# Deltares/xugrid

Hardware: AMD Instinct MI355X
Metric: target cells regridded/s (OverlapRegridder 1M->1M tri, weights + mean apply) (higher is better)
Workload: dtype f64; 1 GPU; BASELINE config 2: ~1M-triangle jittered-lattice Delaunay source -> ~1M-triangle target (seed 1, rotated 30 deg, scaled 0.7), OverlapRegridder area-weighted mean, K=1; target_faces=999660, candidate_pairs=6677422, nnz=4052965, parallelism=1 GPU

## Files before the change

include/xugrid_amd.h:

```cpp
#ifndef XUGRID_AMD_H
#define XUGRID_AMD_H

#include <stdint.h>

#ifdef __cplusplus
extern "C" {
#endif

#define XR_OK 0
#define XR_ERR_INVALID (-1)
#define XR_ERR_NO_DEVICE (-2)
#define XR_ERR_HIP (-3)
#define XR_ERR_LIMIT (-4)

#define XR_MEAN 0
#define XR_HARMONIC_MEAN 1
#define XR_GEOMETRIC_MEAN 2
#define XR_SUM 3
#define XR_MINIMUM 4
#define XR_MAXIMUM 5
#define XR_MODE 6
#define XR_PERCENTILE 7
#define XR_FIRST_ORDER_CONSERVATIVE 8
#define XR_MAX_OVERLAP 9
#define XR_SELECT 10

#define XR_F64 0
#define XR_F32 1
#define XR_I32 2

#define XR_MAX_FACE_NODES 32

typedef struct xr_mesh xr_mesh;
typedef struct xr_csr xr_csr;
typedef struct xr_outer xr_outer;

const char *xr_last_error(void);
int xr_device_count(int *count);
int xr_init(int device);
int xr_current_device(int *device);
int xr_trim_pool(void);
int xr_version(void);
int xr_set_stream(void *hip_stream, int external, int async_dev);
int xr_set_async(int on);
int xr_set_option(const char *name, int64_t value);
int xr_get_option(const char *name, int64_t *value);
int xr_host_copy(void *dst, const void *src, int64_t bytes);
int xr_host_interleave2(const double *x, int64_t x_stride, const double *y, int64_t y_stride, int64_t n, double *out_xy);

int xr_mesh_create(const double *node_xy, int64_t n_node, const void *faces, int faces_itemsize,
                   int64_t n_face, int64_t n_max_node, int64_t fill_value, xr_mesh **out);
int xr_mesh_create_dev(const double *node_xy_dev, int64_t n_node, const void *faces_dev, int faces_itemsize,
                       int64_t n_face, int64_t n_max_node, int64_t fill_value, xr_mesh **out);
int xr_mesh_create_rectilinear(const double *x_vertices, int64_t nx, const double *y_vertices, int64_t ny,
                               xr_mesh **out);
int xr_mesh_destroy(xr_mesh *mesh);
int xr_mesh_info(const xr_mesh *mesh, int64_t *n_node, int64_t *n_face, int64_t *n_max_node);
int xr_mesh_device_bytes(const xr_mesh *mesh, int64_t *bytes);
int xr_mesh_prepare(xr_mesh *mesh);
int xr_mesh_build_index(xr_mesh *mesh);
int xr_mesh_invalidate(xr_mesh *mesh);
int xr_mesh_area(xr_mesh *mesh, double *area_out);
int xr_mesh_centroids(xr_mesh *mesh, double *centroids_out);
int xr_mesh_faces(xr_mesh *mesh, int64_t *faces_out);
int xr_mesh_download(xr_mesh *mesh, double *node_xy_out, int64_t *faces_out);
int xr_mesh_triangulate(xr_mesh *mesh, xr_mesh **out);
int xr_mesh_triangle_face_dev(const xr_mesh *triangles, int64_t *index_dev);
int xr_mesh_circumcenters_dev(xr_mesh *mesh, double *out_dev);
int xr_mesh_perimeter_dev(xr_mesh *mesh, double *out_dev);
int xr_mesh_face_bounds_dev(xr_mesh *mesh, double *out_dev);

int xr_overlap(xr_mesh *tree, xr_mesh *query, int relative, xr_csr **out);
int xr_overlap_stats(const xr_mesh *tree, int64_t *n_candidates);
int xr_overlap_apply_dev(xr_mesh *tree, xr_mesh *query, int relative, int method, double percentile,
                         const void *source_dev, int source_dtype, int64_t K, double *out_dev, xr_csr **out);

int xr_locate_points(xr_mesh *mesh, const double *points, int64_t n, double tolerance,
                     int64_t *face_index_out);
int xr_locate_raster(xr_mesh *mesh, const double *x, int64_t nx, const double *y, int64_t ny,
                     double tolerance, int64_t *face_index_out);
int xr_barycentric(xr_mesh *mesh, const double *points, int64_t n, double tolerance,
                   int64_t *face_index_out, double *weights_out);

int xr_replace_interpolated_weights(const double *vertices, int64_t n_vertex, const int64_t *faces, int64_t n_face,
                                    int64_t m, const int64_t *face_index, double *weights, int64_t n,
                                    const int64_t *node_to_node_map, int64_t n_map);

int xr_locate_csr(xr_mesh *tree, xr_mesh *query, const double *points, int64_t n, double tolerance,
                  xr_csr **out);

int xr_barycentric_csr(xr_mesh *voronoi, xr_mesh *source, xr_mesh *query, const double *points,
                       int64_t n, double tolerance, const int64_t *vertex_face,
                       const int64_t *node_to_node_map, int64_t n_extra, xr_csr **out);
int xr_barycentric_csr_tail(xr_mesh *voronoi, xr_mesh *source, xr_mesh *query, const double *points, int64_t n,
                            double tolerance, int64_t n_identity, const int64_t *vertex_face_tail,
                            const int64_t *node_to_node_map, int64_t n_extra, int tree_order, xr_csr **out);

typedef struct xr_points xr_points;
int xr_locate_flags_begin(xr_mesh *source, xr_mesh *query, const double *points, int64_t n, xr_points **out);
int xr_points_destroy(xr_points *points);
int xr_barycentric_csr_points(xr_mesh *voronoi, xr_mesh *source, xr_points *points, double tolerance, int64_t n_identity,
                              const int64_t *vertex_face_tail, const int64_t *node_to_node_map, int64_t n_extra,
                              int tree_order, xr_csr **out);

typedef struct xr_voronoi xr_voronoi;
int xr_voronoi_create(xr_mesh *mesh, xr_voronoi **out);
int xr_voronoi_create_flags(xr_mesh *mesh, int add_exterior, int add_vertices, int skip_concave, const double *generators_dev,
                            xr_voronoi **out);
int xr_voronoi_vertex_info(const xr_voronoi *v, int64_t *n_generator_vertex, int64_t *max_used_face);
int xr_voronoi_info(const xr_voronoi *v, int64_t *n_node, int64_t *nnz, int64_t *n_exterior_edge,
                    int64_t *n_interior_cell, int64_t *max_interior_degree);
int xr_voronoi_download(const xr_voronoi *v, int64_t *indptr, int64_t *indices, int64_t *edge_nodes,
                        int64_t *edge_face, double *centroids);
int xr_voronoi_boundary_info(xr_voronoi *v, int64_t *n_boundary_node, int64_t *n_boundary_entry);
int xr_voronoi_boundary(xr_voronoi *v, int64_t *nodes, int64_t *row_ptr, int64_t *faces, double *face_xy,
                        int64_t *edge_nodes, int64_t *edge_face, double *edge_face_xy);
int xr_voronoi_mesh(const xr_voronoi *v, const double *extra_xy, int64_t n_extra_vertex,
                    const int64_t *boundary_cells, int64_t n_boundary_cell, int64_t n_max_boundary,
// ... 253 lines not shown
```

xugrid_amd/_lib.py:

```python
import ctypes
import os

_HERE = os.path.dirname(os.path.abspath(__file__))
LIB_PATH = os.environ.get("XUGRID_AMD_LIB") or os.path.join(_HERE, "libxugrid_amd.so")

XR_OK = 0
XR_ERR_INVALID = -1
XR_ERR_NO_DEVICE = -2
XR_ERR_HIP = -3
XR_ERR_LIMIT = -4

XR_F64 = 0
XR_F32 = 1
XR_I32 = 2


class XugridAmdError(RuntimeError):
    """HIP runtime failure, missing device or missing shared library."""


c_i64 = ctypes.c_int64
c_f64 = ctypes.c_double
c_int = ctypes.c_int
vp = ctypes.c_void_p
p_i64 = ctypes.POINTER(ctypes.c_int64)
p_f64 = ctypes.POINTER(ctypes.c_double)
p_int = ctypes.POINTER(ctypes.c_int)
p_vp = ctypes.POINTER(ctypes.c_void_p)

SIGNATURES = {
    "xr_last_error": (ctypes.c_char_p, []),
    "xr_device_count": (c_int, [p_int]),
    "xr_init": (c_int, [c_int]),
    "xr_current_device": (c_int, [p_int]),
    "xr_trim_pool": (c_int, []),
    "xr_version": (c_int, []),
    "xr_set_stream": (c_int, [vp, c_int, c_int]),
    "xr_set_async": (c_int, [c_int]),
    "xr_set_option": (c_int, [ctypes.c_char_p, ctypes.c_int64]),
    "xr_get_option": (c_int, [ctypes.c_char_p, ctypes.POINTER(ctypes.c_int64)]),
    "xr_host_copy": (c_int, [vp, vp, c_i64]),
    "xr_host_interleave2": (c_int, [vp, c_i64, vp, c_i64, c_i64, vp]),
    "xr_mesh_create": (c_int, [vp, c_i64, vp, c_int, c_i64, c_i64, c_i64, p_vp]),
    "xr_mesh_create_dev": (c_int, [vp, c_i64, vp, c_int, c_i64, c_i64, c_i64, p_vp]),
    "xr_mesh_create_rectilinear": (c_int, [vp, c_i64, vp, c_i64, p_vp]),
    "xr_mesh_destroy": (c_int, [vp]),
    "xr_mesh_info": (c_int, [vp, p_i64, p_i64, p_i64]),
    "xr_mesh_device_bytes": (c_int, [vp, p_i64]),
    "xr_mesh_prepare": (c_int, [vp]),
    "xr_mesh_build_index": (c_int, [vp]),
    "xr_mesh_invalidate": (c_int, [vp]),
    "xr_mesh_area": (c_int, [vp, vp]),
    "xr_mesh_centroids": (c_int, [vp, vp]),
    "xr_mesh_faces": (c_int, [vp, vp]),
    "xr_mesh_download": (c_int, [vp, vp, vp]),
    "xr_mesh_triangulate": (c_int, [vp, p_vp]),
    "xr_mesh_triangle_face_dev": (c_int, [vp, vp]),
    "xr_mesh_circumcenters_dev": (c_int, [vp, vp]),
    "xr_mesh_perimeter_dev": (c_int, [vp, vp]),
    "xr_mesh_face_bounds_dev": (c_int, [vp, vp]),
    "xr_voronoi_create": (c_int, [vp, p_vp]),
    "xr_voronoi_create_flags": (c_int, [vp, c_int, c_int, c_int, vp, p_vp]),
    "xr_voronoi_vertex_info": (c_int, [vp, p_i64, p_i64]),
    "xr_voronoi_info": (c_int, [vp, p_i64, p_i64, p_i64, p_i64, p_i64]),
    "xr_voronoi_download": (c_int, [vp, vp, vp, vp, vp, vp]),
    "xr_voronoi_boundary_info": (c_int, [vp, vp, vp]),
    "xr_voronoi_boundary": (c_int, [vp, vp, vp, vp, vp, vp, vp, vp]),
    "xr_voronoi_mesh": (c_int, [vp, vp, c_i64, vp, c_i64, c_i64, p_vp]),
    "xr_voronoi_mesh_auto": (c_int, [vp, p_vp, p_i64, p_i64]),
    "xr_voronoi_tail": (c_int, [vp, vp, vp]),
    "xr_voronoi_boundary_cells_info": (c_int, [vp, p_i64, p_i64, p_i64]),
    "xr_voronoi_boundary_cells": (c_int, [vp, vp, vp]),
    "xr_voronoi_destroy": (c_int, [vp]),
    "xr_overlap": (c_int, [vp, vp, c_int, p_vp]),
    "xr_overlap_stats": (c_int, [vp, p_i64]),
    "xr_overlap_apply_dev": (c_int, [vp, vp, c_int, c_int, c_f64, vp, c_int, c_i64, vp, p_vp]),
    "xr_overlap_partial_dev": (c_int, [vp, vp, c_int, c_int, vp, c_int, c_i64, vp, c_int, p_vp]),
    "xr_shard_plan_dev": (c_int, [vp, vp, c_i64, c_int, vp, vp, c_i64, c_int, c_int, c_int, c_int, vp, p_i64, vp, p_i64, vp]),
    "xr_locate_points": (c_int, [vp, vp, c_i64, c_f64, vp]),
    "xr_locate_raster": (c_int, [vp, vp, c_i64, vp, c_i64, c_f64, vp]),
    "xr_barycentric": (c_int, [vp, vp, c_i64, c_f64, vp, vp]),
    "xr_locate_csr": (c_int, [vp, vp, vp, c_i64, c_f64, p_vp]),
    "xr_replace_interpolated_weights": (c_int, [vp, c_i64, vp, c_i64, c_i64, vp, vp, c_i64, vp, c_i64]),
    "xr_barycentric_csr": (c_int, [vp, vp, vp, vp, c_i64, c_f64, vp, vp, c_i64, p_vp]),
    "xr_barycentric_csr_tail": (c_int, [vp, vp, vp, vp, c_i64, c_f64, c_i64, vp, vp, c_i64, c_int, p_vp]),
    "xr_locate_flags_begin": (c_int, [vp, vp, vp, c_i64, p_vp]),
    "xr_points_destroy": (c_int, [vp]),
    "xr_barycentric_csr_points": (c_int, [vp, vp, vp, c_f64, c_i64, vp, vp, c_i64, c_int, p_vp]),
    "xr_csr_info": (c_int, [vp, p_i64, p_i64, p_i64]),
    "xr_csr_download": (c_int, [vp, vp, vp, vp]),
    "xr_csr_upload": (c_int, [vp, vp, vp, c_i64, c_i64, c_i64, p_vp]),
    "xr_csr_from_triplet": (c_int, [vp, vp, vp, c_i64, c_i64, c_i64, p_vp]),
    "xr_csr_from_outer": (c_int, [vp, vp, vp, c_i64, c_i64, vp, vp, vp, c_i64, c_i64, p_vp]),
    "xr_outer_create": (c_int, [vp, vp, vp, c_i64, c_i64, vp, vp, vp, c_i64, c_i64, p_vp]),
    "xr_outer_info": (c_int, [vp, vp, vp, vp]),
    "xr_outer_csr": (c_int, [vp, p_vp]),
    "xr_outer_destroy": (c_int, [vp]),
    "xr_apply_outer": (c_int, [vp, c_int, c_f64, vp, c_int, c_i64, vp]),
    "xr_apply_outer_dev": (c_int, [vp, c_int, c_f64, vp, c_int, c_i64, vp]),
    "xr_edge_length_csr": (c_int, [vp, vp, c_i64, p_vp]),
    "xr_edge_length_csr_dev": (c_int, [vp, vp, c_i64, p_vp]),
    "xr_edge_pieces": (c_int, [vp, vp, vp, c_i64, vp]),
    "xr_csr_set_row_keys": (c_int, [vp, vp, c_i64]),
    "xr_csr_set_col_keys": (c_int, [vp, vp, c_i64]),
    "xr_csr_col_order": (c_int, [vp, vp]),
    "xr_csr_expect_permuted": (c_int, [vp, c_int]),
    "xr_csr_output_stored_order": (c_int, [vp, c_int]),
    "xr_csr_row_order": (c_int, [vp, c_i64, vp]),
# ... 162 lines not shown
```

xugrid_amd/csrc/xr_agg.h:

```cpp
#pragma once

#include <cstdint>

namespace xr {

static constexpr int AGG_SLOTS = 512;
struct KeyTable {
    int32_t key[AGG_SLOTS];
    int32_t cnt[AGG_SLOTS];
    int32_t base[AGG_SLOTS];
};
__device__ __forceinline__ void agg_clear(KeyTable &t) {
    for (int s = threadIdx.x; s < AGG_SLOTS; s += 256) {
        t.key[s] = -1;
        t.cnt[s] = 0;
    }
}
__device__ __forceinline__ int agg_insert(KeyTable &t, int k, int &rank) {
    int s = (int)(((unsigned)k * 2654435761u) >> 23) & (AGG_SLOTS - 1);
    while (true) {
        const int prev = atomicCAS(&t.key[s], -1, k);
        if (prev == -1 || prev == k) break;
        s = (s + 1) & (AGG_SLOTS - 1);
    }
    rank = atomicAdd(&t.cnt[s], 1);
    return s;
}

}
```

xugrid_amd/csrc/xr_internal.h:

```cpp
#pragma once
#include <memory>

#include <hip/hip_runtime.h>

#include <cstdint>
#include <cstdio>
#include <cstring>
#include <map>
#include <functional>
#include <mutex>
#include <shared_mutex>
#include <string>
#include <type_traits>
#include <vector>

#include "../../include/xugrid_amd.h"

namespace xr {

void set_error(const char *fmt, ...);

struct Failure {
    int code;
};
// ... 225 lines not shown
    OPT_NN_QUERY_SORT,
    OPT_BURN_STRIPS,
    OPT_FACET_TILE,
    OPT_SCAN_FUSED_TILES,
    OPT_MERGE_TABLE_SLACK,
    OPT_FRONT_FUSED,
    OPT_COUNT
};
int64_t option(Option o);

inline unsigned div_up(int64_t a, int64_t b) { return (unsigned)((a + b - 1) / b); }

template <typename F> void with_nodes_per_face(int m, F &&f) {
    if (m == 3) f(std::integral_constant<int, 3>());
    else if (m == 4) f(std::integral_constant<int, 4>());
    else f(std::integral_constant<int, 0>());
}

template <typename F> void with_source_type(int dtype, F &&f) {
    XR_REQUIRE(dtype == XR_F64 || dtype == XR_F32, XR_ERR_INVALID, "unsupported source dtype id %d", dtype);
    if (dtype == XR_F64) f(double());
    else f(float());
}

template <auto KERNEL> void allow_dynamic_lds(size_t bytes) {
    static const bool set = [&] {
        XR_HIP(hipFuncSetAttribute(reinterpret_cast<const void *>(KERNEL), hipFuncAttributeMaxDynamicSharedMemorySize, (int)bytes));
        return true;
    }();
    (void)set;
}

enum class OnFailure { FreeOnly, WaitFirst };
template <typename T> struct Building {
    std::unique_ptr<T> p{new T()};
    OnFailure rule;
    explicit Building(OnFailure r = OnFailure::FreeOnly) : rule(r) {}
    Building(const Building &) = delete;
    Building &operator=(const Building &) = delete;
    ~Building() {
        if (!p || rule != OnFailure::WaitFirst) return;
        try {
            stream_sync();
        } catch (const Failure &) {
        }
    }
    T *operator->() const { return p.get(); }
    T *get() const { return p.get(); }
    T *release() { return p.release(); }
};

void exclusive_scan_i32(const int32_t *in, int32_t *out, int64_t n, int32_t *host_total = nullptr,
                        const int32_t *extra_src = nullptr, int32_t *extra_host = nullptr);
void fill_i32(int32_t *p, int32_t v, int64_t n);
void fill_f64(double *p, double v, int64_t n);

}
```

xugrid_amd/csrc/xr_mesh.hip:

```cpp
#include <algorithm>
#include <cmath>
#include <cstdlib>
#include <vector>

#include <memory>

#include <atomic>

#include "xr_objects.h"
#include "xr_agg.h"
#include "xr_prims.h"

namespace xr {

static constexpr int PREP_BLOCK = 256;

__device__ __forceinline__ double wave_min(double v) {
#pragma unroll
    for (int d = 32; d > 0; d >>= 1) v = fmin(v, __shfl_down(v, d, 64));
    return v;
}
__device__ __forceinline__ double wave_max(double v) {
#pragma unroll
    for (int d = 32; d > 0; d >>= 1) v = fmax(v, __shfl_down(v, d, 64));
// ... 522 lines not shown
    const std::integral_constant<int, 3> m3;
    const std::integral_constant<int, 4> m4;
    if (tree->m == 3) query->m == 3 ? launch(m3, m3) : launch(m3, m4);
    else query->m == 3 ? launch(m4, m3) : launch(m4, m4);
    prepare_done(tree, t_partials.get(), nb_sample, t_tail, true);
    tree->stats_sampled = true;
    host_stamp(1);
    prepare_done(query, q_partials.get(), nb_query, q_tail, true);
}

const double *mesh_area(xr_mesh *mesh) {
    if (mesh->area_valid) return mesh->area.get();
    const int64_t F = mesh->n_face;
    mesh->area.alloc((size_t)F);
    if (F > 0) {
        const dim3 grid(div_up(F, 256)), block(256);
        with_nodes_per_face(mesh->m, [&](auto mc) {
            XR_LAUNCH("face_area", k_face_area<mc()>, grid, block, 0, mesh->node_xy.get(), mesh->faces_raw.get(), F, mesh->m,
                      mesh->area.get());
        });
    }
    mesh->area_valid = true;
    return mesh->area.get();
}

void mesh_read_stats(xr_mesh *mesh, bool need_exact) {
    if (!mesh->prepared) mesh_prepare(mesh, false);
    else if (need_exact && mesh->stats_sampled) mesh_prepare(mesh, mesh->has_attrs, false, false);
    if (mesh->stats_valid) return;
    if (!(mesh->stats_polled && poll_pinned_f64(mesh->stats_host + 8, mesh->stats_seq))) {
        if (mesh->stats_event_pending) XR_HIP(hipEventSynchronize(mesh->stats_event));
        else XR_HIP(hipStreamSynchronize(engine().stream));
        XR_REQUIRE(!mesh->stats_polled || mesh->stats_host[8] == mesh->stats_seq, XR_ERR_HIP, "mesh statistics did not arrive");
    }
    for (int i = 0; i < 8; i++) mesh->h_stats[i] = mesh->stats_host[i];
    mesh->stats_valid = true;
}



__device__ __forceinline__ int face_cell(const GridParams &g, const int32_t *lv, double4 bb) {
    const double e = fmax(bb.y - bb.x, bb.w - bb.z);
    const int l = level_of_extent(g, e);
    const double inv_h = level_inv_h(g, l);
    const int nx = lv[l], ny = lv[MAX_LEVELS + l], base = lv[2 * MAX_LEVELS + l];
    const int cx = cell_coord(bb.x, g.x0, inv_h, nx);
    const int cy = cell_coord(bb.z, g.y0, inv_h, ny);
    return base + cy * nx + cx;
}

template <bool INDEX, int MC>
__global__ void __launch_bounds__(256)
k_spatial_count(const double *__restrict__ node_xy, const int32_t *__restrict__ faces_raw, int64_t n, int m_rt,
                GridParams g, MortonParams mp, int32_t *__restrict__ key, int32_t *__restrict__ count,
                const double *__restrict__ bbox_opt = nullptr ) {
    constexpr int MA = MC > 0 ? MC : XR_MAX_FACE_NODES;
    const int m = MC > 0 ? MC : m_rt;
    __shared__ int32_t sh_lv[3 * MAX_LEVELS];
    if (INDEX) {
        if (threadIdx.x < MAX_LEVELS) {
            sh_lv[threadIdx.x] = g.nx[threadIdx.x];
            sh_lv[MAX_LEVELS + threadIdx.x] = g.ny[threadIdx.x];
            sh_lv[2 * MAX_LEVELS + threadIdx.x] = g.base[threadIdx.x];
        }
        __syncthreads();
    }
    __shared__ KeyTable sh_tab;
    agg_clear(sh_tab);
    __syncthreads();
    const int64_t f = (int64_t)blockIdx.x * 256 + threadIdx.x;
    if (f < n) {
        double xmin = INFINITY, xmax = -INFINITY, ymin = INFINITY, ymax = -INFINITY;
        if (MC == 0 && bbox_opt) {
            const double4 b = reinterpret_cast<const double4 *>(bbox_opt)[f];
            xmin = b.x, xmax = b.y, ymin = b.z, ymax = b.w;
        } else {
            bool open = true;
#pragma unroll
            for (int j = 0; j < MA; j++) {
                if (j < m) {
                    const int v = faces_raw[f * m + j];
                    open = open && !(j >= 3 && v < 0);
                    if (open) {
                        const P2 p = load_p2(node_xy, v);
                        xmin = fmin(xmin, p.x);
                        xmax = fmax(xmax, p.x);
                        ymin = fmin(ymin, p.y);
                        ymax = fmax(ymax, p.y);
                    }
                }
            }
        }
        const double4 bb = make_double4(xmin, xmax, ymin, ymax);
        const int k = INDEX ? face_cell(g, sh_lv, bb) : morton_key(mp, bb);
        key[f] = k;
        int rank;
        agg_insert(sh_tab, k, rank);
    }
    __syncthreads();
    for (int s = threadIdx.x; s < AGG_SLOTS; s += 256)
        if (sh_tab.key[s] >= 0) atomicAdd(&count[sh_tab.key[s]], sh_tab.cnt[s]);
}

template <bool INDEX, int MC>
__global__ void __launch_bounds__(256)
k_spatial_scatter(const int32_t *__restrict__ key, int64_t n, int m_rt, const int32_t *__restrict__ start,
                  int32_t *__restrict__ cursor, const double *__restrict__ node_xy,
                  const int32_t *__restrict__ faces_raw, int32_t *__restrict__ perm, double *__restrict__ o_fxy,
                  uint8_t *__restrict__ o_len, double *__restrict__ o_bbox, float *__restrict__ o_recbb, double x0,
                  double y0, const double *__restrict__ bbox_opt = nullptr, const uint8_t *__restrict__ len_opt = nullptr) {
    constexpr int MA = MC > 0 ? MC : XR_MAX_FACE_NODES;
    const int m = MC > 0 ? MC : m_rt;
    const int64_t f = (int64_t)blockIdx.x * 256 + threadIdx.x;
    __shared__ KeyTable sh_tab;
    agg_clear(sh_tab);
    const bool valid = f < n;
    const bool stored_only = MC == 0 && bbox_opt && len_opt && !o_fxy;
    int face[MA];
    if (valid && !stored_only) {
#pragma unroll
        for (int j = 0; j < MA; j++)
            if (j < m) face[j] = faces_raw[f * m + j];
    }
    const int k = valid ? key[f] : -1;
    __syncthreads();
    int tab_slot = 0, rank = 0;
    if (valid) tab_slot = agg_insert(sh_tab, k, rank);
    __syncthreads();
    for (int s = threadIdx.x; s < AGG_SLOTS; s += 256)
        if (sh_tab.key[s] >= 0) sh_tab.base[s] = start[sh_tab.key[s]] + atomicSub(&cursor[sh_tab.key[s]], sh_tab.cnt[s]) - sh_tab.cnt[s];
    __syncthreads();
    if (!valid) return;
    const int64_t r = (int64_t)sh_tab.base[tab_slot] + rank;
    if (stored_only) {
        const double4 b = reinterpret_cast<const double4 *>(bbox_opt)[f];
        perm[r] = (int32_t)f;
        o_len[r] = len_opt[f];
        if (INDEX)
            reinterpret_cast<float4 *>(o_recbb)[r] = make_float4(f32_below(b.x - x0), f32_above(b.y - x0), f32_below(b.z - y0), f32_above(b.w - y0));
        else
            reinterpret_cast<double4 *>(o_bbox)[r] = b;
        return;
    }
    int nl;
    bool flip;
    face_shape<MA>(node_xy, face, m, nl, flip);
    constexpr bool PREFETCH = MC > 0;
    P2 pts[PREFETCH ? MA : 1];
    if (PREFETCH) {
#pragma unroll
        for (int j = 0; j < MA; j++)
            if (j < nl) pts[j] = load_p2(node_xy, face[j]);
    }
    perm[r] = (int32_t)f;
    o_len[r] = (uint8_t)nl;
    double2 *dst = reinterpret_cast<double2 *>(o_fxy) + r * m;
    double xmin = INFINITY, xmax = -INFINITY, ymin = INFINITY, ymax = -INFINITY;
#pragma unroll
    for (int j = 0; j < MA; j++) {
        if (j < nl) {
            const P2 p = PREFETCH ? pts[PREFETCH ? j : 0] : load_p2(node_xy, face[j]);
            xmin = fmin(xmin, p.x);
            xmax = fmax(xmax, p.x);
            ymin = fmin(ymin, p.y);
            ymax = fmax(ymax, p.y);
            if (o_fxy) dst[flip ? nl - 1 - j : j] = make_double2(p.x, p.y);
        }
    }
    if (INDEX) {
        reinterpret_cast<float4 *>(o_recbb)[r] =
            make_float4(f32_below(xmin - x0), f32_above(xmax - x0), f32_below(ymin - y0), f32_above(ymax - y0));
    } else if (o_bbox) {
        reinterpret_cast<double4 *>(o_bbox)[r] = make_double4(xmin, xmax, ymin, ymax);
    }
}

template <bool INDEX>
static void spatial_sort(xr_mesh *mesh, const GridParams &g, const MortonParams &mp, int64_t n_buckets,
                         int32_t *bucket_start, int32_t *perm, double *o_fxy, uint8_t *o_len, double *o_bbox,
                         float *o_recbb) {
    const int64_t F = mesh->n_face;
    const double *boxes = mesh->has_attrs && mesh->m != 3 && mesh->m != 4 ? mesh->bbox.get() : nullptr;
    const uint8_t *lens = boxes ? mesh->len.get() : nullptr;
    DevBuf<int32_t> key((size_t)F), count_own;
    int32_t *count = zero_scratch(0, (size_t)n_buckets);
    const bool cached = count != nullptr;
    if (!cached) {
        count_own.alloc((size_t)n_buckets);
        count = count_own.get();
        XR_HIP(hipMemsetAsync(count, 0, sizeof(int32_t) * (((size_t)n_buckets + 3) & ~(size_t)3), launch_stream()));
    }
    if (F > 0) {
        const char *name = INDEX ? "index_count" : "order_count";
        const dim3 grid(div_up(F, 256)), block(256);
        with_nodes_per_face(mesh->m, [&](auto mc) {
            XR_LAUNCH(name, (k_spatial_count<INDEX, mc()>), grid, block, 0, mesh->node_xy.get(), mesh->faces_raw.get(), F,
                      mesh->m, g, mp, key.get(), count, boxes);
        });
    }
    exclusive_scan_i32(count, bucket_start, n_buckets);
    if (F > 0) {
        const char *name = INDEX ? "index_scatter" : "order_scatter";
        const dim3 grid(div_up(F, 256)), block(256);
        with_nodes_per_face(mesh->m, [&](auto mc) {
            XR_LAUNCH(name, (k_spatial_scatter<INDEX, mc()>), grid, block, 0, key.get(), F, mesh->m, bucket_start, count,
                      mesh->node_xy.get(), mesh->faces_raw.get(), perm, o_fxy, o_len, o_bbox, o_recbb, g.x0, g.y0, boxes, lens);
        });
    }
    if (cached) zero_scratch_done(0);
}

void mesh_query_order(xr_mesh *mesh) {
    if (mesh->query_ready) return;
    mesh_read_stats(mesh, true);
    const int64_t F = mesh->n_face;
    const int m = mesh->m;
    const double mean_ext = F > 0 ? mesh->h_stats[4] / (double)F : 0.0;
    const double mean_jump = F > 0 ? mesh->h_stats[7] / ((double)F * 63.0 / 64.0) : 0.0;
    mesh->query_identity = F == 0 || mean_jump <= 4.0 * mean_ext;
    if (mesh->query_identity) {
        mesh_face_coords(mesh);
        mesh->query_ready = true;
        return;
    }
    mesh->q_perm.alloc((size_t)F);
    if (!mesh->ragged()) mesh->q_fxy.alloc((size_t)F * m * 2);
    mesh->q_len.alloc((size_t)F);
    if (mesh->ragged()) mesh->q_bbox.alloc((size_t)F * 4);
    if (F > 0) {
        const double xmin = mesh->h_stats[0], xmax = mesh->h_stats[1], ymin = mesh->h_stats[2], ymax = mesh->h_stats[3];
        double span = std::max(xmax - xmin, ymax - ymin);
        if (!(span > 0)) span = 1.0;
        double h = 2.0 * mesh->h_stats[4] / (double)F;
        if (!(h > 0)) h = span;
        int bits = 1;
        while (bits < 10 && ldexp(h, bits) < span) bits++;
        MortonParams mp{xmin, ymin, (double)(1 << bits) / (span * (1.0 + 1e-9)), 1 << bits};
        GridParams g{};
        DevBuf<int32_t> start(((size_t)1 << (2 * bits)) + 1);
        spatial_sort<false>(mesh, g, mp, (int64_t)1 << (2 * bits), start.get(), mesh->q_perm.get(),
                            mesh->ragged() ? (double *)nullptr : mesh->q_fxy.get(), mesh->q_len.get(), mesh->q_bbox.get(),
                            nullptr);
    }
    if (mesh->ragged()) ragged_fill(mesh, mesh->q_perm.get(), mesh->q_len.get(), mesh->q_off, mesh->q_fxy);
    mesh->query_ready = true;
}

void mesh_build_index(xr_mesh *mesh) {
    if (mesh->indexed) return;
    mesh_read_stats(mesh);
    const int64_t F = mesh->n_face;
    const int m = mesh->m;
    XR_REQUIRE(F < (int64_t)1 << 31, XR_ERR_LIMIT, "mesh has too many faces for int32 indices");
    const double xmin = mesh->h_stats[0], xmax = mesh->h_stats[1], ymin = mesh->h_stats[2], ymax = mesh->h_stats[3];
    const bool sampled = mesh->stats_sampled;
    const double n_ext = sampled ? std::max(mesh->h_stats[7], 1.0) : (double)F;
    const double sum_ext = mesh->h_stats[4] * ((double)F / n_ext);
    const double max_ext = sampled ? std::max(xmax - xmin, ymax - ymin) : mesh->h_stats[5];
    GridParams g{};
// ... 525 lines not shown
    tri->n_face = n_triangle;
    tri->m = 3;
    tri->is_triangulation = true;
    tri->node_xy.alloc((size_t)N * 2);
    tri->faces_raw.alloc((size_t)n_triangle * 3);
    tri->tri_face.alloc((size_t)n_triangle);
    if (N > 0)
        XR_HIP(hipMemcpyAsync(tri->node_xy.get(), mesh->node_xy.get(), sizeof(double) * 2 * (size_t)N, hipMemcpyDeviceToDevice,
                              launch_stream()));
    if (n_triangle > 0)
        XR_LAUNCH("tri_scatter", k_tri_scatter, dim3(div_up(F * 3 * (m - 2), 256)), dim3(256), 0, mesh->faces_raw.get(), F, m,
                  m == 3 ? (const int32_t *)nullptr : off.get(), tri->faces_raw.get(), tri->tri_face.get());
    stream_sync();
    *out = tri.release();
    XR_API_END
}

int xr_mesh_triangle_face_dev(const xr_mesh *triangles, int64_t *index_dev) {
    XR_API_BEGIN
    XR_REQUIRE(triangles && (index_dev || triangles->n_face == 0), XR_ERR_INVALID, "xr_mesh_triangle_face_dev: NULL argument");
    XR_REQUIRE(triangles->is_triangulation, XR_ERR_INVALID, "xr_mesh_triangle_face_dev: the mesh was not made by xr_mesh_triangulate");
    widen_dev(triangles->tri_face.get(), triangles->n_face, index_dev);
    dev_call_done();
    XR_API_END
}

int xr_mesh_faces(xr_mesh *mesh, int64_t *faces_out) {
    XR_API_BEGIN
    XR_REQUIRE(mesh && faces_out, XR_ERR_INVALID, "xr_mesh_faces: NULL argument");
    const int64_t n = mesh->n_face * mesh->m;
    if (n > 0) {
        DevBuf<int64_t> wide((size_t)n);
        XR_LAUNCH("faces_ccw", k_faces_ccw, dim3(div_up(mesh->n_face, 256)), dim3(256), 0, mesh->node_xy.get(),
                  mesh->faces_raw.get(), mesh->n_face, mesh->m, wide.get(), false);
        d2h(faces_out, wide.get(), sizeof(int64_t) * (size_t)n);
        stream_sync();
    }
    XR_API_END
}

int xr_mesh_download(xr_mesh *mesh, double *node_xy_out, int64_t *faces_out) {
    XR_API_BEGIN
    XR_REQUIRE(mesh, XR_ERR_INVALID, "xr_mesh_download: NULL handle");
    if (node_xy_out && mesh->n_node > 0) d2h(node_xy_out, mesh->node_xy.get(), sizeof(double) * 2 * (size_t)mesh->n_node);
    const int64_t n = mesh->n_face * mesh->m;
    if (faces_out && n > 0) {
        std::vector<int32_t> raw((size_t)n);
        d2h(raw.data(), mesh->faces_raw.get(), sizeof(int32_t) * (size_t)n);
        for (int64_t i = 0; i < n; i++) faces_out[i] = raw[(size_t)i];
    }
    XR_API_END
}

}
```

xugrid_amd/csrc/xr_scan.hip:

```cpp
#include "xr_internal.h"
#include "xr_prims.h"

namespace xr {

static constexpr int SCAN_BLOCK = 256;
static constexpr int SCAN_ITEMS = 8;
static constexpr int SCAN_TILE = SCAN_BLOCK * SCAN_ITEMS;

__device__ __forceinline__ void load_items(const int32_t *__restrict__ in, int64_t base, int64_t n, int (&v)[SCAN_ITEMS]) {
    static_assert(SCAN_ITEMS == 8, "two int4 per thread");
    if (base + SCAN_ITEMS <= n && (reinterpret_cast<uintptr_t>(in) & 15) == 0) {
        const int4 a = *reinterpret_cast<const int4 *>(in + base), b = *reinterpret_cast<const int4 *>(in + base + 4);
        v[0] = a.x; v[1] = a.y; v[2] = a.z; v[3] = a.w;
        v[4] = b.x; v[5] = b.y; v[6] = b.z; v[7] = b.w;
    } else {
#pragma unroll
        for (int i = 0; i < SCAN_ITEMS; i++) v[i] = base + i < n ? in[base + i] : 0;
    }
}
__device__ __forceinline__ void store_scanned(int32_t *__restrict__ out, int64_t base, int64_t n, const int (&v)[SCAN_ITEMS], int ex) {
    int o[SCAN_ITEMS];
#pragma unroll
    for (int i = 0; i < SCAN_ITEMS; i++) {
        o[i] = ex;
        ex += v[i];
    }
    if (base + SCAN_ITEMS <= n && (reinterpret_cast<uintptr_t>(out) & 15) == 0) {
        *reinterpret_cast<int4 *>(out + base) = make_int4(o[0], o[1], o[2], o[3]);
        *reinterpret_cast<int4 *>(out + base + 4) = make_int4(o[4], o[5], o[6], o[7]);
    } else {
#pragma unroll
        for (int i = 0; i < SCAN_ITEMS; i++)
            if (base + i < n) out[base + i] = o[i];
    }
}

__global__ void __launch_bounds__(SCAN_BLOCK) k_scan_reduce(const int32_t *__restrict__ in,
                                                            int32_t *__restrict__ block_sums, int64_t n) {
    __shared__ int lds[4];
    const int64_t base = (int64_t)blockIdx.x * SCAN_TILE;
    int s = 0;
#pragma unroll
    for (int i = 0; i < SCAN_ITEMS; i++) {
        int64_t j = base + (int64_t)i * SCAN_BLOCK + threadIdx.x;
        if (j < n) s += in[j];
    }
    int tot;
    (void)block_excl_scan(s, &tot, lds);
    if (threadIdx.x == 0) block_sums[blockIdx.x] = tot;
}

__global__ void __launch_bounds__(SCAN_BLOCK) k_scan_partials(int32_t *__restrict__ sums, int64_t nb,
                                                              int32_t *__restrict__ total_out, int32_t *host_total,
                                                              const int32_t *extra_src, int32_t *extra_host) {
    __shared__ int lds[4];
    int carry = 0;
    for (int64_t base = 0; base < nb; base += SCAN_BLOCK) {
        int64_t j = base + threadIdx.x;
        int v = j < nb ? sums[j] : 0;
        int tot;
        int ex = block_excl_scan(v, &tot, lds);
        if (j < nb) sums[j] = carry + ex;
        carry += tot;
    }
    if (threadIdx.x == 0 && total_out) *total_out = carry;
    if (threadIdx.x == 0 && host_total) *host_total = carry;
    if (threadIdx.x == 0 && extra_host) *extra_host = *extra_src;
}

__global__ void __launch_bounds__(SCAN_BLOCK) k_scan_apply(const int32_t *__restrict__ in,
                                                           const int32_t *__restrict__ block_off,
                                                           int32_t *__restrict__ out, int64_t n) {
    __shared__ int lds[4];
    const int64_t base = (int64_t)blockIdx.x * SCAN_TILE + (int64_t)threadIdx.x * SCAN_ITEMS;
    int v[SCAN_ITEMS];
    load_items(in, base, n, v);
    int s = 0;
#pragma unroll
    for (int i = 0; i < SCAN_ITEMS; i++) s += v[i];
    int tot;
    const int ex = block_excl_scan(s, &tot, lds) + block_off[blockIdx.x];
    store_scanned(out, base, n, v, ex);
}

__global__ void k_fill_i32(int32_t *p, int32_t v, int64_t n) {
    int64_t i = (int64_t)blockIdx.x * blockDim.x + threadIdx.x;
    if (i < n) p[i] = v;
}
__global__ void k_fill_f64(double *p, double v, int64_t n) {
    int64_t i = (int64_t)blockIdx.x * blockDim.x + threadIdx.x;
    if (i < n) p[i] = v;
}

static constexpr int SCAN_FUSED_TILES = 8192;

__global__ void __launch_bounds__(SCAN_BLOCK) k_scan_apply_fused(const int32_t *__restrict__ in,
                                                                 const int32_t *__restrict__ tile_sums, int64_t nb,
                                                                 int32_t *__restrict__ out, int64_t n, int32_t *host_total,
                                                                 const int32_t *extra_src, int32_t *extra_host) {
    __shared__ int lds[4];
    __shared__ int sh_base;
    int part = 0;
    for (int64_t i = threadIdx.x; i < blockIdx.x; i += SCAN_BLOCK) part += tile_sums[i];
    int tot;
    (void)block_excl_scan(part, &tot, lds);
    if (threadIdx.x == 0) sh_base = tot;
    __syncthreads();
    const int64_t base = (int64_t)blockIdx.x * SCAN_TILE + (int64_t)threadIdx.x * SCAN_ITEMS;
    int v[SCAN_ITEMS];
    load_items(in, base, n, v);
    int s = 0;
#pragma unroll
    for (int i = 0; i < SCAN_ITEMS; i++) s += v[i];
    const int ex = block_excl_scan(s, &tot, lds) + sh_base;
    store_scanned(out, base, n, v, ex);
    if (blockIdx.x == nb - 1 && threadIdx.x == 0) {
        out[n] = sh_base + tot;
        if (host_total) *host_total = sh_base + tot;
        if (extra_host) *extra_host = *extra_src;
    }
}

void exclusive_scan_i32(const int32_t *in, int32_t *out, int64_t n, int32_t *host_total, const int32_t *extra_src,
                        int32_t *extra_host) {
    if (n <= 0) {
        fill_i32(out, 0, 1);
        if (host_total) {
            stream_sync();
            *host_total = 0;
            if (extra_host) d2h(extra_host, extra_src, sizeof(int32_t));
        }
        return;
    }
    const int64_t nb = (n + SCAN_TILE - 1) / SCAN_TILE;
    DevBuf<int32_t> sums((size_t)nb);
    XR_LAUNCH("scan_reduce", k_scan_reduce, dim3((unsigned)nb), dim3(SCAN_BLOCK), 0, in, sums.get(), n);
    const int64_t fused_tiles = option(OPT_SCAN_FUSED_TILES) > 0 ? option(OPT_SCAN_FUSED_TILES) : SCAN_FUSED_TILES;
    if (nb <= fused_tiles) {
        XR_LAUNCH("scan_apply", k_scan_apply_fused, dim3((unsigned)nb), dim3(SCAN_BLOCK), 0, in, sums.get(), nb, out, n,
                  host_total, extra_src, extra_host);
        return;
    }
    XR_LAUNCH("scan_partials", k_scan_partials, dim3(1), dim3(SCAN_BLOCK), 0, sums.get(), nb, out + n, host_total, extra_src,
              extra_host);
    XR_LAUNCH("scan_apply", k_scan_apply, dim3((unsigned)nb), dim3(SCAN_BLOCK), 0, in, sums.get(), out, n);
}

void fill_i32(int32_t *p, int32_t v, int64_t n) {
    if (n <= 0) return;
    XR_LAUNCH("fill_i32", k_fill_i32, dim3(div_up(n, 256)), dim3(256), 0, p, v, n);
}
void fill_f64(double *p, double v, int64_t n) {
    if (n <= 0) return;
    XR_LAUNCH("fill_f64", k_fill_f64, dim3(div_up(n, 256)), dim3(256), 0, p, v, n);
}

}
```

xugrid_amd/engine.py:

```python
import ctypes

import numpy as np

from . import _lib
from ._lib import XR_F32, XR_F64, check

IntDType = np.intp
FloatDType = np.float64

METHOD_IDS = {
    "mean": 0,
    "harmonic_mean": 1,
    "geometric_mean": 2,
    "sum": 3,
    "minimum": 4,
    "maximum": 5,
    "mode": 6,
    "percentile": 7,
    "first_order_conservative": 8,
    "conductance": 8,
    "max_overlap": 9,
    "select": 10,
}

# ... 238 lines not shown
    @classmethod
    def from_rectilinear(cls, x_vertices, y_vertices):
        xv = np.ascontiguousarray(x_vertices, dtype=np.float64)
        yv = np.ascontiguousarray(y_vertices, dtype=np.float64)
        if xv.ndim != 1 or yv.ndim != 1 or xv.size < 2 or yv.size < 2:
            raise ValueError("x_vertices and y_vertices must be 1-D arrays of at least two vertices")
        handle = ctypes.c_void_p()
        check(_lib.load().xr_mesh_create_rectilinear(_ptr(xv), xv.size - 1, _ptr(yv), yv.size - 1, ctypes.byref(handle)))
        return cls._from_handle(handle)

    @classmethod
    def from_device(cls, node_xy_ptr, n_node, faces_ptr, faces_itemsize, n_face, n_max_node, fill_value=-1):
        handle = ctypes.c_void_p()
        check(
            _lib.load().xr_mesh_create_dev(
                ctypes.c_void_p(int(node_xy_ptr)), int(n_node), ctypes.c_void_p(int(faces_ptr)), int(faces_itemsize),
                int(n_face), int(n_max_node), int(fill_value), ctypes.byref(handle),
            )
        )
        self = cls.__new__(cls)
        self._h = handle
        self.n_node, self.n_face, self.n_max_node = int(n_node), int(n_face), int(n_max_node)
        return self

    def download(self):
        xy = np.empty((self.n_node, 2), dtype=np.float64)
        faces = np.empty((self.n_face, self.n_max_node), dtype=np.int64)
        check(_lib.load().xr_mesh_download(self._h, _ptr(xy), _ptr(faces)))
        return xy, faces

    def __init__(self, vertices, faces, fill_value=-1):
        lib = _lib.load()
        xy = _as_xy(vertices)
        f = _as_faces(faces)
        self.n_node = xy.shape[0]
        self.n_face, self.n_max_node = f.shape
        handle = ctypes.c_void_p()
        check(
            lib.xr_mesh_create(
                _ptr(xy), self.n_node, _ptr(f), f.dtype.itemsize, self.n_face, self.n_max_node,
                int(fill_value), ctypes.byref(handle),
            )
        )
        self._h = handle

    def prepare(self):
        check(_lib.load().xr_mesh_prepare(self._h))

    def build_index(self):
        check(_lib.load().xr_mesh_build_index(self._h))

    def invalidate(self):
        check(_lib.load().xr_mesh_invalidate(self._h))

    def device_bytes(self):
        n = ctypes.c_int64(0)
        check(_lib.load().xr_mesh_device_bytes(self._h, ctypes.byref(n)))
        return n.value

    def area(self):
        out = np.empty(self.n_face, dtype=np.float64)
        check(_lib.load().xr_mesh_area(self._h, _ptr(out)))
        return out

    def centroids(self):
        out = np.empty((self.n_face, 2), dtype=np.float64)
        check(_lib.load().xr_mesh_centroids(self._h, _ptr(out)))
        return out

    def faces_ccw(self):
        out = np.empty((self.n_face, self.n_max_node), dtype=np.int64)
        check(_lib.load().xr_mesh_faces(self._h, _ptr(out)))
        return out

    def triangulate(self) -> "DeviceMesh":
        handle = ctypes.c_void_p()
        check(_lib.load().xr_mesh_triangulate(self._h, ctypes.byref(handle)))
        return DeviceMesh._from_handle(handle)

    def triangle_face_dev(self, like=None):
        out, ptr = empty_like_device(like, (self.n_face,), np.int64)
        check(_lib.load().xr_mesh_triangle_face_dev(self._h, ctypes.c_void_p(ptr)))
        return out

    def _derived_dev(self, name, shape):
        out = DeviceArray(shape, np.float64)
        check(getattr(_lib.load(), name)(self._h, ctypes.c_void_p(out.ptr)))
        return out

    def circumcenters_dev(self) -> "DeviceArray":
        if self.n_max_node != 3:
            raise NotImplementedError("Circumcenters are only supported for triangular grids")
        return self._derived_dev("xr_mesh_circumcenters_dev", (self.n_face, 2))

    def perimeter_dev(self) -> "DeviceArray":
        return self._derived_dev("xr_mesh_perimeter_dev", (self.n_face,))

    def face_bounds_dev(self) -> "DeviceArray":
        return self._derived_dev("xr_mesh_face_bounds_dev", (self.n_face, 4))

    def subset(self, face_index_ptr, n):
        handle, identity, problems = ctypes.c_void_p(), ctypes.c_int(), (ctypes.c_int64 * 2)()
        check(_lib.load().xr_mesh_subset_dev(self._h, ctypes.c_void_p(int(face_index_ptr)), int(n), ctypes.byref(handle),
                                             ctypes.byref(identity), problems))
        mesh = DeviceMesh._from_handle(handle) if handle.value else None
        return mesh, bool(identity.value), (int(problems[0]), int(problems[1]))
# ... 893 lines not shown
```

Measured before the change: 2.149 billion target cells/s.

## Fuse bucket rank assignment into count kernel and reuse per-tile sums in scan

The spatial count kernel now records each face's final rank within its bucket by taking the bucket base from the global atomicAdd, so the scatter kernel no longer rebuilds a shared hash table or uses atomic cursors. The count kernel also accumulates per-scan-tile sums, with striped words to reduce contention, which lets the scan skip its reduce pass. The scan clears the histogram as it reads it, so the separate zeroing step goes away. This adds an int2 key array, extra shared-memory tables and atomics in the count kernel. It also adds an index_view debug API.

```diff
diff --git a/include/xugrid_amd.h b/include/xugrid_amd.h
--- a/include/xugrid_amd.h
+++ b/include/xugrid_amd.h
@@ -64,6 +64,7 @@
 int xr_mesh_centroids(xr_mesh *mesh, double *centroids_out);
 int xr_mesh_faces(xr_mesh *mesh, int64_t *faces_out);
 int xr_mesh_download(xr_mesh *mesh, double *node_xy_out, int64_t *faces_out);
+int xr_mesh_index_view(xr_mesh *mesh, int64_t *sizes_out, int32_t *cell_start_out, int32_t *rec_face_out, int32_t *level_base_out);
 int xr_mesh_triangulate(xr_mesh *mesh, xr_mesh **out);
 int xr_mesh_triangle_face_dev(const xr_mesh *triangles, int64_t *index_dev);
 int xr_mesh_circumcenters_dev(xr_mesh *mesh, double *out_dev);
diff --git a/xugrid_amd/_lib.py b/xugrid_amd/_lib.py
--- a/xugrid_amd/_lib.py
+++ b/xugrid_amd/_lib.py
@@ -54,6 +54,7 @@
     "xr_mesh_centroids": (c_int, [vp, vp]),
     "xr_mesh_faces": (c_int, [vp, vp]),
     "xr_mesh_download": (c_int, [vp, vp, vp]),
+    "xr_mesh_index_view": (c_int, [vp, vp, vp, vp, vp]),
     "xr_mesh_triangulate": (c_int, [vp, p_vp]),
     "xr_mesh_triangle_face_dev": (c_int, [vp, vp]),
     "xr_mesh_circumcenters_dev": (c_int, [vp, vp]),
diff --git a/xugrid_amd/csrc/xr_agg.h b/xugrid_amd/csrc/xr_agg.h
--- a/xugrid_amd/csrc/xr_agg.h
+++ b/xugrid_amd/csrc/xr_agg.h
@@ -27,4 +27,24 @@
     return s;
 }
 
+struct TileTable {
+    int32_t key[AGG_SLOTS];
+    int32_t cnt[AGG_SLOTS];
+};
+__device__ __forceinline__ void agg_clear(TileTable &t) {
+    for (int s = threadIdx.x; s < AGG_SLOTS; s += 256) {
+        t.key[s] = -1;
+        t.cnt[s] = 0;
+    }
 }
+__device__ __forceinline__ void agg_add(TileTable &t, int k, int n) {
+    int s = (int)(((unsigned)k * 2654435761u) >> 23) & (AGG_SLOTS - 1);
+    while (true) {
+        const int prev = atomicCAS(&t.key[s], -1, k);
+        if (prev == -1 || prev == k) break;
+        s = (s + 1) & (AGG_SLOTS - 1);
+    }
+    atomicAdd(&t.cnt[s], n);
+}
+
+}
diff --git a/xugrid_amd/csrc/xr_internal.h b/xugrid_amd/csrc/xr_internal.h
--- a/xugrid_amd/csrc/xr_internal.h
+++ b/xugrid_amd/csrc/xr_internal.h
@@ -301,6 +301,15 @@
 
 void exclusive_scan_i32(const int32_t *in, int32_t *out, int64_t n, int32_t *host_total = nullptr,
                         const int32_t *extra_src = nullptr, int32_t *extra_host = nullptr);
+static constexpr int SCAN_TILE = 2048;
+static constexpr int SCAN_SUM_WORDS = 8, SCAN_SUM_STRIDE = 32;
+__host__ __device__ inline int64_t tile_sum_word(int64_t tile, unsigned part) {
+    return (tile * SCAN_SUM_WORDS + (part & (SCAN_SUM_WORDS - 1))) * SCAN_SUM_STRIDE;
+}
+inline int64_t tile_sum_words(int64_t tiles) { return tiles * SCAN_SUM_WORDS * SCAN_SUM_STRIDE; }
+int64_t scan_tiles(int64_t n);
+bool scan_tiles_given(int64_t n);
+void exclusive_scan_tiles_i32(int32_t *in, const int32_t *tile_sums, int32_t *out, int64_t n);
 void fill_i32(int32_t *p, int32_t v, int64_t n);
 void fill_f64(double *p, double v, int64_t n);
 
diff --git a/xugrid_amd/csrc/xr_mesh.hip b/xugrid_amd/csrc/xr_mesh.hip
--- a/xugrid_amd/csrc/xr_mesh.hip
+++ b/xugrid_amd/csrc/xr_mesh.hip
@@ -598,7 +598,9 @@
 template <bool INDEX, int MC>
 __global__ void __launch_bounds__(256)
 k_spatial_count(const double *__restrict__ node_xy, const int32_t *__restrict__ faces_raw, int64_t n, int m_rt,
-                GridParams g, MortonParams mp, int32_t *__restrict__ key, int32_t *__restrict__ count,
+                GridParams g, MortonParams mp, int2 *__restrict__ key_rank ,
+                int32_t *__restrict__ count,
+                int32_t *__restrict__ tile_sums ,
                 const double *__restrict__ bbox_opt = nullptr ) {
     constexpr int MA = MC > 0 ? MC : XR_MAX_FACE_NODES;
     const int m = MC > 0 ? MC : m_rt;
@@ -612,9 +614,12 @@
         __syncthreads();
     }
     __shared__ KeyTable sh_tab;
+    __shared__ TileTable sh_tiles;
     agg_clear(sh_tab);
+    if (tile_sums) agg_clear(sh_tiles);
     __syncthreads();
     const int64_t f = (int64_t)blockIdx.x * 256 + threadIdx.x;
+    int k = -1, tab_slot = 0, rank = 0;
     if (f < n) {
         double xmin = INFINITY, xmax = -INFINITY, ymin = INFINITY, ymax = -INFINITY;
         if (MC == 0 && bbox_opt) {
@@ -638,46 +643,49 @@
             }
         }
         const double4 bb = make_double4(xmin, xmax, ymin, ymax);
-        const int k = INDEX ? face_cell(g, sh_lv, bb) : morton_key(mp, bb);
-        key[f] = k;
-        int rank;
-        agg_insert(sh_tab, k, rank);
+        k = INDEX ? face_cell(g, sh_lv, bb) : morton_key(mp, bb);
+        tab_slot = agg_insert(sh_tab, k, rank);
     }
     __syncthreads();
-    for (int s = threadIdx.x; s < AGG_SLOTS; s += 256)
-        if (sh_tab.key[s] >= 0) atomicAdd(&count[sh_tab.key[s]], sh_tab.cnt[s]);
+    for (int s = threadIdx.x; s < AGG_SLOTS; s += 256) {
+        const int sk = sh_tab.key[s];
+        if (sk < 0) continue;
+        const int c = sh_tab.cnt[s];
+        sh_tab.base[s] = atomicAdd(&count[sk], c);
+        if (tile_sums) agg_add(sh_tiles, sk / SCAN_TILE, c);
+    }
+    __syncthreads();
+    if (tile_sums) {
+        for (int s = threadIdx.x; s < AGG_SLOTS; s += 256)
+            if (sh_tiles.key[s] >= 0) atomicAdd(&tile_sums[tile_sum_word(sh_tiles.key[s], blockIdx.x)], sh_tiles.cnt[s]);
+    }
+    if (f < n) key_rank[f] = make_int2(k, sh_tab.base[tab_slot] + rank);
 }
 
 template <bool INDEX, int MC>
 __global__ void __launch_bounds__(256)
-k_spatial_scatter(const int32_t *__restrict__ key, int64_t n, int m_rt, const int32_t *__restrict__ start,
-                  int32_t *__restrict__ cursor, const double *__restrict__ node_xy,
+k_spatial_scatter(const int2 *__restrict__ key_rank, int64_t n, int m_rt, const int32_t *__restrict__ start,
+                  int32_t *__restrict__ hist, const double *__restrict__ node_xy,
                   const int32_t *__restrict__ faces_raw, int32_t *__restrict__ perm, double *__restrict__ o_fxy,
                   uint8_t *__restrict__ o_len, double *__restrict__ o_bbox, float *__restrict__ o_recbb, double x0,
-                  double y0, const double *__restrict__ bbox_opt = nullptr, const uint8_t *__restrict__ len_opt = nullptr) {
+                  double y0, int32_t *__restrict__ tile_sums, int64_t n_tiles, bool clear_hist,
+                  const double *__restrict__ bbox_opt = nullptr, const uint8_t *__restrict__ len_opt = nullptr) {
     constexpr int MA = MC > 0 ? MC : XR_MAX_FACE_NODES;
     const int m = MC > 0 ? MC : m_rt;
     const int64_t f = (int64_t)blockIdx.x * 256 + threadIdx.x;
-    __shared__ KeyTable sh_tab;
-    agg_clear(sh_tab);
-    const bool valid = f < n;
+    if (blockIdx.x == 0 && tile_sums)
+        for (int64_t i = threadIdx.x; i < n_tiles * SCAN_SUM_WORDS; i += 256) tile_sums[i * SCAN_SUM_STRIDE] = 0;
+    if (f >= n) return;
     const bool stored_only = MC == 0 && bbox_opt && len_opt && !o_fxy;
     int face[MA];
-    if (valid && !stored_only) {
+    if (!stored_only) {
 #pragma unroll
         for (int j = 0; j < MA; j++)
             if (j < m) face[j] = faces_raw[f * m + j];
     }
-    const int k = valid ? key[f] : -1;
-    __syncthreads();
-    int tab_slot = 0, rank = 0;
-    if (valid) tab_slot = agg_insert(sh_tab, k, rank);
-    __syncthreads();
-    for (int s = threadIdx.x; s < AGG_SLOTS; s += 256)
-        if (sh_tab.key[s] >= 0) sh_tab.base[s] = start[sh_tab.key[s]] + atomicSub(&cursor[sh_tab.key[s]], sh_tab.cnt[s]) - sh_tab.cnt[s];
-    __syncthreads();
-    if (!valid) return;
-    const int64_t r = (int64_t)sh_tab.base[tab_slot] + rank;
+    const int2 kr = key_rank[f];
+    const int64_t r = (int64_t)start[kr.x] + kr.y;
+    if (clear_hist) hist[kr.x] = 0;
     if (stored_only) {
         const double4 b = reinterpret_cast<const double4 *>(bbox_opt)[f];
         perm[r] = (int32_t)f;
@@ -728,29 +736,37 @@
     const int64_t F = mesh->n_face;
     const double *boxes = mesh->has_attrs && mesh->m != 3 && mesh->m != 4 ? mesh->bbox.get() : nullptr;
     const uint8_t *lens = boxes ? mesh->len.get() : nullptr;
-    DevBuf<int32_t> key((size_t)F), count_own;
-    int32_t *count = zero_scratch(0, (size_t)n_buckets);
+    const bool tile_scan = scan_tiles_given(n_buckets);
+    const int64_t n_tiles = tile_scan ? scan_tiles(n_buckets) : 0;
+    const size_t hist_words = ((size_t)n_buckets + SCAN_SUM_STRIDE - 1) & ~(size_t)(SCAN_SUM_STRIDE - 1);
+    const size_t n_words = hist_words + (size_t)tile_sum_words(n_tiles);
+    DevBuf<int2> key_rank((size_t)F);
+    DevBuf<int32_t> count_own;
+    int32_t *count = zero_scratch(0, n_words);
     const bool cached = count != nullptr;
     if (!cached) {
-        count_own.alloc((size_t)n_buckets);
+        count_own.alloc(n_words);
         count = count_own.get();
-        XR_HIP(hipMemsetAsync(count, 0, sizeof(int32_t) * (((size_t)n_buckets + 3) & ~(size_t)3), launch_stream()));
-    }
+        XR_HIP(hipMemsetAsync(count, 0, sizeof(int32_t) * ((n_words + 3) & ~(size_t)3), launch_stream()));
+    }
+    int32_t *tile_sums = tile_scan ? count + hist_words : nullptr;
     if (F > 0) {
         const char *name = INDEX ? "index_count" : "order_count";
         const dim3 grid(div_up(F, 256)), block(256);
         with_nodes_per_face(mesh->m, [&](auto mc) {
             XR_LAUNCH(name, (k_spatial_count<INDEX, mc()>), grid, block, 0, mesh->node_xy.get(), mesh->faces_raw.get(), F,
-                      mesh->m, g, mp, key.get(), count, boxes);
+                      mesh->m, g, mp, key_rank.get(), count, tile_sums, boxes);
         });
     }
-    exclusive_scan_i32(count, bucket_start, n_buckets);
+    if (tile_scan) exclusive_scan_tiles_i32(count, tile_sums, bucket_start, n_buckets);
+    else exclusive_scan_i32(count, bucket_start, n_buckets);
     if (F > 0) {
         const char *name = INDEX ? "index_scatter" : "order_scatter";
         const dim3 grid(div_up(F, 256)), block(256);
         with_nodes_per_face(mesh->m, [&](auto mc) {
-            XR_LAUNCH(name, (k_spatial_scatter<INDEX, mc()>), grid, block, 0, key.get(), F, mesh->m, bucket_start, count,
-                      mesh->node_xy.get(), mesh->faces_raw.get(), perm, o_fxy, o_len, o_bbox, o_recbb, g.x0, g.y0, boxes, lens);
+            XR_LAUNCH(name, (k_spatial_scatter<INDEX, mc()>), grid, block, 0, key_rank.get(), F, mesh->m, bucket_start, count,
+                      mesh->node_xy.get(), mesh->faces_raw.get(), perm, o_fxy, o_len, o_bbox, o_recbb, g.x0, g.y0, tile_sums,
+                      n_tiles, !tile_scan, boxes, lens);
         });
     }
     if (cached) zero_scratch_done(0);
@@ -1382,4 +1398,20 @@
     XR_API_END
 }
 
-}
+int xr_mesh_index_view(xr_mesh *mesh, int64_t *sizes_out, int32_t *cell_start_out, int32_t *rec_face_out, int32_t *level_base_out) {
+    XR_API_BEGIN
+    XR_REQUIRE(mesh && sizes_out, XR_ERR_INVALID, "xr_mesh_index_view: NULL argument");
+    mesh_build_index(mesh);
+    const GridParams &g = mesh->grid;
+    sizes_out[0] = g.n_cells;
+    sizes_out[1] = g.n_levels;
+    sizes_out[2] = mesh->n_face;
+    if (cell_start_out) d2h(cell_start_out, mesh->cell_start.get(), sizeof(int32_t) * ((size_t)g.n_cells + 1));
+    if (rec_face_out && mesh->n_face > 0) d2h(rec_face_out, mesh->rec_face.get(), sizeof(int32_t) * (size_t)mesh->n_face);
+    if (level_base_out)
+        for (int l = 0; l < g.n_levels; l++) level_base_out[l] = g.base[l];
+    stream_sync();
+    XR_API_END
+}
+
+}
diff --git a/xugrid_amd/csrc/xr_scan.hip b/xugrid_amd/csrc/xr_scan.hip
--- a/xugrid_amd/csrc/xr_scan.hip
+++ b/xugrid_amd/csrc/xr_scan.hip
@@ -5,7 +5,7 @@
 
 static constexpr int SCAN_BLOCK = 256;
 static constexpr int SCAN_ITEMS = 8;
-static constexpr int SCAN_TILE = SCAN_BLOCK * SCAN_ITEMS;
+static_assert(SCAN_TILE == SCAN_BLOCK * SCAN_ITEMS, "a tile is what one block scans (SCAN_TILE: xr_internal.h)");
 
 __device__ __forceinline__ void load_items(const int32_t *__restrict__ in, int64_t base, int64_t n, int (&v)[SCAN_ITEMS]) {
     static_assert(SCAN_ITEMS == 8, "two int4 per thread");
@@ -94,14 +94,19 @@
 
 static constexpr int SCAN_FUSED_TILES = 8192;
 
-__global__ void __launch_bounds__(SCAN_BLOCK) k_scan_apply_fused(const int32_t *__restrict__ in,
+template <bool GIVEN>
+__global__ void __launch_bounds__(SCAN_BLOCK) k_scan_apply_fused(std::conditional_t<GIVEN, int32_t *, const int32_t *__restrict__> in,
                                                                  const int32_t *__restrict__ tile_sums, int64_t nb,
                                                                  int32_t *__restrict__ out, int64_t n, int32_t *host_total,
                                                                  const int32_t *extra_src, int32_t *extra_host) {
     __shared__ int lds[4];
     __shared__ int sh_base;
     int part = 0;
-    for (int64_t i = threadIdx.x; i < blockIdx.x; i += SCAN_BLOCK) part += tile_sums[i];
+    if constexpr (GIVEN) {
+        for (int64_t i = threadIdx.x; i < (int64_t)blockIdx.x * SCAN_SUM_WORDS; i += SCAN_BLOCK) part += tile_sums[i * SCAN_SUM_STRIDE];
+    } else {
+        for (int64_t i = threadIdx.x; i < blockIdx.x; i += SCAN_BLOCK) part += tile_sums[i];
+    }
     int tot;
     (void)block_excl_scan(part, &tot, lds);
     if (threadIdx.x == 0) sh_base = tot;
@@ -114,6 +119,16 @@
     for (int i = 0; i < SCAN_ITEMS; i++) s += v[i];
     const int ex = block_excl_scan(s, &tot, lds) + sh_base;
     store_scanned(out, base, n, v, ex);
+    if constexpr (GIVEN) {
+        if (base + SCAN_ITEMS <= n && (reinterpret_cast<uintptr_t>(in) & 15) == 0) {
+            *reinterpret_cast<int4 *>(in + base) = make_int4(0, 0, 0, 0);
+            *reinterpret_cast<int4 *>(in + base + 4) = make_int4(0, 0, 0, 0);
+        } else {
+#pragma unroll
+            for (int i = 0; i < SCAN_ITEMS; i++)
+                if (base + i < n) in[base + i] = 0;
+        }
+    }
     if (blockIdx.x == nb - 1 && threadIdx.x == 0) {
         out[n] = sh_base + tot;
         if (host_total) *host_total = sh_base + tot;
@@ -137,13 +152,28 @@
     XR_LAUNCH("scan_reduce", k_scan_reduce, dim3((unsigned)nb), dim3(SCAN_BLOCK), 0, in, sums.get(), n);
     const int64_t fused_tiles = option(OPT_SCAN_FUSED_TILES) > 0 ? option(OPT_SCAN_FUSED_TILES) : SCAN_FUSED_TILES;
     if (nb <= fused_tiles) {
-        XR_LAUNCH("scan_apply", k_scan_apply_fused, dim3((unsigned)nb), dim3(SCAN_BLOCK), 0, in, sums.get(), nb, out, n,
+        XR_LAUNCH("scan_apply", k_scan_apply_fused<false>, dim3((unsigned)nb), dim3(SCAN_BLOCK), 0, in, sums.get(), nb, out, n,
                   host_total, extra_src, extra_host);
         return;
     }
     XR_LAUNCH("scan_partials", k_scan_partials, dim3(1), dim3(SCAN_BLOCK), 0, sums.get(), nb, out + n, host_total, extra_src,
               extra_host);
     XR_LAUNCH("scan_apply", k_scan_apply, dim3((unsigned)nb), dim3(SCAN_BLOCK), 0, in, sums.get(), out, n);
+}
+
+int64_t scan_tiles(int64_t n) { return (n + SCAN_TILE - 1) / SCAN_TILE; }
+
+static constexpr int SCAN_GIVEN_TILES = 1024;
+bool scan_tiles_given(int64_t n) {
+    const int64_t fused_tiles = option(OPT_SCAN_FUSED_TILES) > 0 ? option(OPT_SCAN_FUSED_TILES) : SCAN_FUSED_TILES;
+    return n > 0 && scan_tiles(n) <= std::min<int64_t>(fused_tiles, SCAN_GIVEN_TILES);
+}
+
+void exclusive_scan_tiles_i32(int32_t *in, const int32_t *tile_sums, int32_t *out, int64_t n) {
+    XR_REQUIRE(scan_tiles_given(n) && in != out, XR_ERR_INVALID, "exclusive_scan_tiles_i32: %lld elements are not a fused scan", (long long)n);
+    const int64_t nb = scan_tiles(n);
+    XR_LAUNCH("scan_apply", k_scan_apply_fused<true>, dim3((unsigned)nb), dim3(SCAN_BLOCK), 0, in, tile_sums, nb, out, n,
+              (int32_t *)nullptr, (const int32_t *)nullptr, (int32_t *)nullptr);
 }
 
 void fill_i32(int32_t *p, int32_t v, int64_t n) {
diff --git a/xugrid_amd/engine.py b/xugrid_amd/engine.py
--- a/xugrid_amd/engine.py
+++ b/xugrid_amd/engine.py
@@ -314,6 +314,18 @@
 
     def invalidate(self):
         check(_lib.load().xr_mesh_invalidate(self._h))
+
+    def index_view(self):
+        lib = _lib.load()
+        sizes = np.zeros(3, dtype=np.int64)
+        check(lib.xr_mesh_index_view(self._h, _ptr(sizes), None, None, None))
+        n_cells, n_levels, n_face = (int(v) for v in sizes)
+        cell_start = np.empty(n_cells + 1, dtype=np.int32)
+        rec_face = np.empty(n_face, dtype=np.int32)
+        level_base = np.empty(n_levels, dtype=np.int32)
+        check(lib.xr_mesh_index_view(self._h, _ptr(sizes), _ptr(cell_start), _ptr(rec_face), _ptr(level_base)))
+        return dict(n_cells=n_cells, n_levels=n_levels, n_face=n_face, cell_start=cell_start, rec_face=rec_face,
+                    level_base=level_base)
 
     def device_bytes(self):
         n = ctypes.c_int64(0)
```

Result: faster. 2.183 billion target cells/s, median of 5 (+1.6%).
